# masnottuh/point-cloud-toolbox

Measured on AMD Instinct MI355X. Metric: points/sec curvature (1M-pt torus, k=50); HBM GB/s k-NN vs peak, higher is better.
Workload: dtype f64

## Files before the change

### point-cloud-toolbox_amd/csrc/pct_knn.hip

```cpp
#include "pct_knn_sweep.h"

namespace {

constexpr unsigned kPadElem = 0xFFFFFFFFu;

template <int R>
struct FastK {
    unsigned e[R];
};

__device__ __forceinline__ unsigned umed3(unsigned a, unsigned b, unsigned c) {
    unsigned r;
    asm("v_med3_u32 %0, %1, %2, %3" : "=v"(r) : "v"(a), "v"(b), "v"(c));
    return r;
}

struct SortLanes {
    unsigned sel[6];
    int a31, a63;
};

__device__ __forceinline__ SortLanes make_sort_lanes() {
    SortLanes c;
    const int lane = lane_id();
// ... 1887 lines not shown
        if (a.stats && lane == 0) atomicAdd(&a.counters[4], (unsigned long long)cnt);
    }
}

__global__ __launch_bounds__(256) void k_plain_records(const float* __restrict__ xyz, int64_t n, float4* __restrict__ out) {
    const int64_t i = (int64_t)blockIdx.x * 256 + threadIdx.x;
    if (i < n) out[i] = make_float4(xyz[3 * i], xyz[3 * i + 1], xyz[3 * i + 2], __int_as_float((int)i));
}

template <int R>
__global__ __launch_bounds__(64 * kWavesPerBlock) void k_query_points(const float4* __restrict__ pts, int n, const double* __restrict__ q_xyz,
                                                                      int64_t m, int k, double eps2, int* __restrict__ idx_out,
                                                                      double* __restrict__ dist_out) {
    __shared__ double s_pend_d[kWavesPerBlock][64 * R + 64];
    __shared__ int s_pend_p[kWavesPerBlock][64 * R + 64];
    const int w = __builtin_amdgcn_readfirstlane(threadIdx.x >> 6);
    const int lane = lane_id();
    const int64_t q = (int64_t)blockIdx.x * kWavesPerBlock + w;
    if (q >= m) return;
    Sweep<R> sw;
    sw.k = k - 1;
    sw.eps2 = eps2;
    sw.pts = pts;
    sw.pend_d = s_pend_d[w];
    sw.pend_p = s_pend_p[w];
    sw.qx = q_xyz[3 * q]; sw.qy = q_xyz[3 * q + 1]; sw.qz = q_xyz[3 * q + 2];
    sw.reset();
    for (int base = 0;; base += 64) {
        const bool have = base < n;
        if (have) {
            const int pos = base + lane;
            const bool valid = pos < n;
            float4 c = make_float4(0.f, 0.f, 0.f, 0.f);
            if (valid) c = pts[pos];
            sw.consider(c, pos, valid);
            if (sw.npend < 64 * R) continue;
        }
        if (sw.npend > 0 || sw.empty) sw.flush();
        if (!have) break;
    }
#pragma unroll
    for (int r = 0; r < R; ++r) {
        const int i = lane + 64 * r;
        if (i < k) {
            const bool real = sw.best.p[r] != INT_MAX;
            idx_out[q * k + i] = real ? sw.best.p[r] : n;
            dist_out[q * k + i] = real ? sqrt(sw.best.d[r]) : (double)INFINITY;
        }
    }
}

__device__ __forceinline__ float table_distance(const float4* pts, const double4* ptsd, int qpos, const float4 c) {
    double qx, qy, qz;
    if (ptsd) { const double4 q = ptsd[qpos]; qx = q.x; qy = q.y; qz = q.z; }
    else { const float4 q = pts[qpos]; qx = (double)q.x; qy = (double)q.y; qz = (double)q.z; }
    const double dx = (double)c.x - qx, dy = (double)c.y - qy, dz = (double)c.z - qz;
    return (float)sqrt((dx * dx + dy * dy) + dz * dz);
}

__global__ __launch_bounds__(256) void k_export(const float4* __restrict__ pts, const double4* __restrict__ ptsd, const int* __restrict__ owned_pos, int q_begin,
                                                const int* __restrict__ nbr_pos, const float* __restrict__ nbr_dist,
                                                const int* __restrict__ nbr_cnt, int64_t n, int64_t n_rows, int k, int pitch,
                                                int64_t begin, int64_t end, int* __restrict__ idx_out,
                                                float* __restrict__ dist_out, int* __restrict__ cnt_out) {
    const int64_t t = (int64_t)blockIdx.x * 256 + threadIdx.x;
    const int64_t row = t / k;
    const int j = (int)(t - row * k);
    if (row >= n_rows) return;
    const int pub = owned_pos ? __float_as_int(pts[owned_pos[row]].w) : (int)row + q_begin;
    if (pub < begin || pub >= end) return;
    const int64_t o = (int64_t)(pub - begin) * k + j;
    const int pos = nbr_pos[row * pitch + j];
    const float4 c = pos < 0 ? make_float4(0.f, 0.f, 0.f, 0.f) : pts[pos];
    if (idx_out) idx_out[o] = pos < 0 ? (int)n : __float_as_int(c.w);
    if (dist_out) dist_out[o] = nbr_dist ? nbr_dist[row * pitch + j] : pos < 0 ? INFINITY : table_distance(pts, ptsd, owned_pos[row], c);
    if (cnt_out && j == 0) cnt_out[pub - begin] = nbr_cnt ? nbr_cnt[row] : k;
}

__global__ __launch_bounds__(128) void k_export_rows(const float4* __restrict__ pts, const double4* __restrict__ ptsd, const int* __restrict__ row_of, const int* __restrict__ owned_pos, int q_begin,
                                                     const int* __restrict__ nbr_pos, const float* __restrict__ nbr_dist,
                                                     const int* __restrict__ nbr_cnt, int64_t n, int k, int pitch,
                                                     const int64_t* __restrict__ rows, int* __restrict__ idx_out,
                                                     float* __restrict__ dist_out, int* __restrict__ cnt_out) {
    const int64_t r = blockIdx.x;
    const int64_t pub = rows[r];
    const int64_t row = row_of ? row_of[pub - q_begin] : pub - q_begin;
    for (int j = threadIdx.x; j < k; j += 128) {
        const int pos = nbr_pos[row * pitch + j];
        const float4 c = pos < 0 ? make_float4(0.f, 0.f, 0.f, 0.f) : pts[pos];
        if (idx_out) idx_out[r * k + j] = pos < 0 ? (int)n : __float_as_int(c.w);
        if (dist_out) dist_out[r * k + j] = nbr_dist ? nbr_dist[row * pitch + j] : pos < 0 ? INFINITY : table_distance(pts, ptsd, owned_pos[row], c);
    }
    if (cnt_out && threadIdx.x == 0) cnt_out[r] = nbr_cnt ? nbr_cnt[row] : k;
}

__global__ __launch_bounds__(64) void k_selftest(int* fails) {
    const int lane = lane_id();
    const int v = lane * 7919 + 13;
    int bad = 0;
    bad += lane_xor<1>(v) != __shfl_xor(v, 1);
    bad += lane_xor<2>(v) != __shfl_xor(v, 2);
    bad += lane_xor<4>(v) != __shfl_xor(v, 4);
    bad += lane_xor<8>(v) != __shfl_xor(v, 8);
    bad += lane_xor<16>(v) != __shfl_xor(v, 16);
    bad += lane_xor<32>(v) != __shfl_xor(v, 32);
    if (bad) atomicAdd(fails, bad);
}

__global__ __launch_bounds__(256) void k_item_census(const int2* __restrict__ items, int64_t n_items, int items_q,
                                                     const int* __restrict__ cs, const int* __restrict__ cell_own, pct_grid g, int k,
                                                     int cap, unsigned long long* __restrict__ out) {
    __shared__ unsigned long long sh[4][4];
    unsigned long long v[4] = {0, 0, 0, 0};
    for (int64_t it = (int64_t)blockIdx.x * 256 + threadIdx.x; it < n_items; it += (int64_t)gridDim.x * 256) {
        const int2 e = items[it];
        const int cell = e.x;
        const int cx = cell % g.nx, cy = (cell / g.nx) % g.ny, cz = cell / (g.nx * g.ny);
        const int nq = min(items_q, cell_own[cell] - e.y * items_q);
        int m = 0, occupied = 0;
        for (int dz = -1; dz <= 1; ++dz)
            for (int dy = -1; dy <= 1; ++dy) {
                const int z = cz + dz, y = cy + dy;
                if (z < 0 || z >= g.nz || y < 0 || y >= g.ny) continue;
                const int row = (z * g.ny + y) * g.nx;
                int prev = cs[row + max(cx - 1, 0)];
                for (int x = max(cx - 1, 0); x <= min(cx + 1, g.nx - 1); ++x) {
                    const int next = cs[row + x + 1];
                    occupied += next > prev;
                    m += next - prev;
                    prev = next;
                }
            }
        v[0] += (unsigned)nq;
        if (m > cap) v[1] += (unsigned)nq;
        else if (2 * m < 5 * (k + 1)) v[2] += (unsigned)nq;
        else v[3] += (unsigned long long)nq * (unsigned)occupied;
    }
    for (int j = 0; j < 4; ++j) {
        for (int o = 32; o > 0; o >>= 1) v[j] += __shfl_xor(v[j], o);
        if ((threadIdx.x & 63) == 0) sh[threadIdx.x >> 6][j] = v[j];
    }
    __syncthreads();
    if (threadIdx.x < 4) atomicAdd(&out[threadIdx.x], sh[0][threadIdx.x] + sh[1][threadIdx.x] + sh[2][threadIdx.x] + sh[3][threadIdx.x]);
}

KnnArgs make_args(pct_ctx* ctx, int32_t k, double eps, bool grid) {
    KnnArgs a = {};
    a.pts = (const float4*)(grid ? ctx->sorted4.p : ctx->pts4.p);
    a.ptsd = ctx->has_f64 ? (const double4*)(grid ? ctx->sorted4d.p : ctx->pts4d.p) : nullptr;
    a.cell_start = (const int*)ctx->cell_cnt.p;
    a.cell_own = (const int*)ctx->cell_own.p;
    a.own_start = (const int*)ctx->own_start.p;
    a.owned_pos = (const int*)ctx->owned_pos.p;
    a.n_owned = ctx->own_flag ? ctx->own_count : ctx->q_end - ctx->q_begin;
    a.occ = (const int*)ctx->occ.p;
    a.n_occ = ctx->n_occ;
    a.n = ctx->n;
    a.g = ctx->grid;
    a.k = k;
    a.pitch = (k + 3) & ~3;
    a.eps2 = eps > 0 ? eps * eps : INFINITY;
    a.q_begin = (int)ctx->q_begin;
    a.q_end = (int)ctx->q_end;
    a.nbr_pos = (int*)ctx->nbr_pos.p;
    a.nbr_dist = (float*)ctx->nbr_dist.p;
    a.nbr_cnt = eps > 0 ? (int*)ctx->nbr_cnt.p : nullptr;
    a.row_done = ctx->own_flag || ctx->level_mode ? (int*)ctx->row_done.p : nullptr;
    a.redo_m = a.row_done ? (int*)ctx->redo_m.p : nullptr;
    a.counters = (unsigned long long*)ctx->counters.p;
    a.stats = ctx->collect_stats ? 1 : 0;
    return a;
}

int reserve_table(pct_ctx* ctx, int32_t k, double eps, bool with_dist = true) {
    ctx->nbr_pitch = (k + 3) & ~3;
    const size_t rows = (size_t)(ctx->own_flag ? ctx->own_count : ctx->q_end - ctx->q_begin);
    PCT_TRY(pct_reserve(ctx, &ctx->nbr_pos, rows * ctx->nbr_pitch * sizeof(int)));
    if (with_dist) PCT_TRY(pct_reserve(ctx, &ctx->nbr_dist, rows * ctx->nbr_pitch * sizeof(float)));
    ctx->dist_valid = with_dist;
    if (eps > 0) PCT_TRY(pct_reserve(ctx, &ctx->nbr_cnt, rows * sizeof(int)));
    PCT_TRY(pct_reserve(ctx, &ctx->counters, 64 * sizeof(unsigned long long)));
    if (!ctx->counters_clean) PCT_HIP(ctx, hipMemsetAsync(ctx->counters.p, 0, 64, ctx->stream));
    ctx->counters_clean = false;
    return PCT_OK;
}

}

int pct_launch_knn_grid(pct_ctx* ctx, int32_t k, double eps, bool exact_only, int phase) {
    const int64_t n_rows = ctx->own_flag ? ctx->own_count : ctx->q_end - ctx->q_begin;
    const double c2_ = ctx->grid.cell * ctx->grid.cell;
    const bool f32_ok_ = c2_ > 1e-30 && c2_ < 1e30 && (!(eps > 0) || eps * eps > 1e-36);
    const pct_grid& gg_ = ctx->grid;
    const double far_ = fmax(fmax(fabs(gg_.ox), fabs(gg_.ox + gg_.nx * gg_.cell)),
                             fmax(fmax(fabs(gg_.oy), fabs(gg_.oy + gg_.ny * gg_.cell)), fmax(fabs(gg_.oz), fabs(gg_.oz + gg_.nz * gg_.cell))));
    const bool q64_ok_ = !ctx->has_f64 || far_ * 0x1p-23 < gg_.cell * 0x1p-7;
    const bool pair_kernel = !exact_only && phase == 0 && q64_ok_ && f32_ok_ && !ctx->own_flag && !ctx->level_mode && ctx->n_items > 0 &&
                             k + 1 <= pct_fast_r1_max() && ctx->n_items < ((int64_t)1 << 31) - 8 && !pct_getenv("PCT_NO_PAIR") &&
                             !pct_getenv("PCT_NO_PAIR_KERNEL");
    const bool duo_kernel = !exact_only && phase == 0 && q64_ok_ && f32_ok_ && !ctx->own_flag && !ctx->level_mode && ctx->n_items > 0 &&
                            k + 1 > pct_fast_r1_max() && k + 1 <= 128 && ctx->n_items < ((int64_t)1 << 31) - 8 &&
                            !pct_getenv("PCT_NO_PAIR") && !pct_getenv("PCT_NO_DUO_KERNEL");
    const bool skip_dist = (pair_kernel || duo_kernel) && ctx->skip_dist_req && !pct_getenv("PCT_KEEP_DIST");
    if (phase != 2) {
        PCT_TRY(reserve_table(ctx, k, eps, !skip_dist));
        PCT_TRY(pct_reserve(ctx, &ctx->redo, ((size_t)n_rows + 16) * sizeof(int)));
        if (ctx->level_mode) PCT_TRY(pct_reserve(ctx, &ctx->redo_m, ((size_t)n_rows + 16) * sizeof(int)));
    }
    KnnArgs a = make_args(ctx, k, eps, true);
    if (!ctx->dist_valid) a.nbr_dist = nullptr;
    int* redo_count = (int*)ctx->counters.p + 14;
    int* redo = (int*)ctx->redo.p;
    const dim3 block(64 * kWavesPerBlock);
    if (!exact_only && phase != 2 && ctx->n_items > 0) {
        const dim3 grid1((unsigned)((ctx->n_items + kFastWaves<1> - 1) / kFastWaves<1>)), block1(64 * kFastWaves<1>);
        const dim3 grid2((unsigned)((ctx->n_items + kFastWaves<2> - 1) / kFastWaves<2>)), block2(64 * kFastWaves<2>);
        const int2* items = (const int2*)ctx->occ.p;
        const double c2 = ctx->grid.cell * ctx->grid.cell;
        const bool f32_ok = c2 > 1e-30 && c2 < 1e30 && (!(eps > 0) || eps * eps > 1e-36);
        const pct_grid& gg = ctx->grid;
        const double far = fmax(fmax(fabs(gg.ox), fabs(gg.ox + gg.nx * gg.cell)),
                                fmax(fmax(fabs(gg.oy), fabs(gg.oy + gg.ny * gg.cell)), fmax(fabs(gg.oz), fabs(gg.oz + gg.nz * gg.cell))));
        const bool q64_ok = ctx->has_f64 && f32_ok && far * 0x1p-23 < gg.cell * 0x1p-7 && !ctx->level_mode;
        const bool e = eps > 0, pre = !ctx->has_f64 && f32_ok, r1 = k + 1 <= pct_fast_r1_max();
#define PCT_FAST(R_, E_, P_, GRID_, BLOCK_) \
    PCT_LAUNCH((k_knn_fast<R_, E_, P_>), GRID_, BLOCK_, 0, ctx->stream, a, items, ctx->n_items, ctx->items_q, redo, redo_count)
        const bool no_pair = pct_getenv("PCT_NO_PAIR") != nullptr;
#define PCT_FAST_PAIR(R_, E_, GRID_, BLOCK_) \
    PCT_LAUNCH((k_knn_fast<R_, E_, true, true>), GRID_, BLOCK_, 0, ctx->stream, a, items, ctx->n_items, ctx->items_q, redo, redo_count)
#define PCT_FAST_PAIR64(R_, E_, GRID_, BLOCK_) \
    PCT_LAUNCH((k_knn_fast<R_, E_, true, true, true>), GRID_, BLOCK_, 0, ctx->stream, a, items, ctx->n_items, ctx->items_q, redo, redo_count)
        if (pair_kernel || duo_kernel) {
            PairArgs pa = {};
            pa.pts = a.pts; pa.ptsd = a.ptsd; pa.cell_start = a.cell_start; pa.cell_own = a.cell_own; pa.own_start = a.own_start;
            pa.items = items;
            pa.nbr_pos = a.nbr_pos; pa.nbr_dist = a.nbr_dist; pa.nbr_cnt = a.nbr_cnt;
            pa.redo = redo; pa.redo_count = redo_count; pa.counters = a.counters;
            pa.n_items = (int)ctx->n_items; pa.items_q = ctx->items_q;
            pa.k = a.k; pa.pitch = a.pitch; pa.stats = a.stats; pa.eps2 = a.eps2; pa.g = a.g;
            const auto magic = [](unsigned d, unsigned* mg, int* sh) {
                int l = 0;
                while ((1ull << l) < d) ++l;
                *sh = 30 + l;
                *mg = (unsigned)(((1ull << *sh) + d - 1) / d);
            };
            magic((unsigned)a.g.nx, &pa.magic_x, &pa.shift_x);
            magic((unsigned)a.g.nx * (unsigned)a.g.ny, &pa.magic_xy, &pa.shift_xy);
            pa.items_per_xcd = (int)((ctx->n_items + 7) / 8);
            if (pct_getenv("PCT_NO_XCD_MAP")) pa.items_per_xcd = 0;
            const int64_t n_blk = pa.items_per_xcd ? (int64_t)pa.items_per_xcd * 8 : ctx->n_items;
            const dim3 gridp((unsigned)((n_blk + kPairWaves - 1) / kPairWaves)), blockp(64 * kPairWaves);
            if (duo_kernel) {
                const dim3 gridd((unsigned)n_blk), blockd(64);
                if (ctx->has_f64) {
                    if (e && skip_dist) PCT_LAUNCH((k_knn_duo<true, false, true>), gridd, blockd, 0, ctx->stream, pa);
                    else if (e) PCT_LAUNCH((k_knn_duo<true, true, true>), gridd, blockd, 0, ctx->stream, pa);
                    else if (skip_dist) PCT_LAUNCH((k_knn_duo<false, false, true>), gridd, blockd, 0, ctx->stream, pa);
                    else PCT_LAUNCH((k_knn_duo<false, true, true>), gridd, blockd, 0, ctx->stream, pa);
                } else
                if (e && skip_dist) PCT_LAUNCH((k_knn_duo<true, false>), gridd, blockd, 0, ctx->stream, pa);
                else if (e) PCT_LAUNCH((k_knn_duo<true, true>), gridd, blockd, 0, ctx->stream, pa);
                else if (skip_dist) PCT_LAUNCH((k_knn_duo<false, false>), gridd, blockd, 0, ctx->stream, pa);
                else PCT_LAUNCH((k_knn_duo<false, true>), gridd, blockd, 0, ctx->stream, pa);
            } else
            if (ctx->has_f64) {
                if (e && skip_dist) PCT_LAUNCH((k_knn_pair<true, false, true>), gridp, blockp, 0, ctx->stream, pa);
                else if (e) PCT_LAUNCH((k_knn_pair<true, true, true>), gridp, blockp, 0, ctx->stream, pa);
                else if (skip_dist) PCT_LAUNCH((k_knn_pair<false, false, true>), gridp, blockp, 0, ctx->stream, pa);
                else PCT_LAUNCH((k_knn_pair<false, true, true>), gridp, blockp, 0, ctx->stream, pa);
            } else
            if (e && skip_dist) PCT_LAUNCH((k_knn_pair<true, false>), gridp, blockp, 0, ctx->stream, pa);
            else if (e) PCT_LAUNCH((k_knn_pair<true, true>), gridp, blockp, 0, ctx->stream, pa);
            else if (skip_dist) PCT_LAUNCH((k_knn_pair<false, false>), gridp, blockp, 0, ctx->stream, pa);
            else PCT_LAUNCH((k_knn_pair<false, true>), gridp, blockp, 0, ctx->stream, pa);
        } else
        if (q64_ok && !no_pair) {
            if (r1 && !e) PCT_FAST_PAIR64(1, false, grid1, block1);
            else if (r1) PCT_FAST_PAIR64(1, true, grid1, block1);
            else if (!e) PCT_FAST_PAIR64(2, false, grid2, block2);
            else PCT_FAST_PAIR64(2, true, grid2, block2);
        } else
        if (r1 && !e && pre && !no_pair) PCT_FAST_PAIR(1, false, grid1, block1);
        else if (r1 && e && pre && !no_pair) PCT_FAST_PAIR(1, true, grid1, block1);
        else if (!r1 && !e && pre && !no_pair) PCT_FAST_PAIR(2, false, grid2, block2);
        else if (!r1 && e && pre && !no_pair) PCT_FAST_PAIR(2, true, grid2, block2);
        else if (r1 && !e && pre) PCT_FAST(1, false, true, grid1, block1);
        else if (r1 && e && pre) PCT_FAST(1, true, true, grid1, block1);
        else if (r1 && !e) PCT_FAST(1, false, false, grid1, block1);
        else if (r1) PCT_FAST(1, true, false, grid1, block1);
        else if (!e && pre) PCT_FAST(2, false, true, grid2, block2);
        else if (e && pre) PCT_FAST(2, true, true, grid2, block2);
        else if (!e) PCT_FAST(2, false, false, grid2, block2);
        else PCT_FAST(2, true, false, grid2, block2);
#undef PCT_FAST
#undef PCT_FAST_PAIR
#undef PCT_FAST_PAIR64
        PCT_HIP(ctx, hipGetLastError());
    }
    PCT_HIP(ctx, hipEventRecord(ctx->ev[7], ctx->stream));
    if (phase != 1) {
        const int64_t waves = exact_only ? n_rows : 32768;
        const int blocks = (int)((waves + kWavesPerBlock - 1) / kWavesPerBlock);
        const int* list = exact_only ? nullptr : redo;
        if (k + 1 <= 64)
            PCT_LAUNCH(k_knn_exact<1>, dim3(blocks), block, 0, ctx->stream, a, list, (const int*)redo_count);
        else if (k + 1 <= 128)
            PCT_LAUNCH(k_knn_exact<2>, dim3(blocks), block, 0, ctx->stream, a, list, (const int*)redo_count);
        else
            PCT_TRY(pct_launch_knn_exact_wide(ctx, a, blocks, list, (const int*)redo_count));
        PCT_HIP(ctx, hipGetLastError());
    }
    ctx->knn_sorted_space = true;
    return PCT_OK;
}

int pct_launch_knn_tree(pct_ctx* ctx, int32_t k, double eps) {
    if (ctx->level_mode || ctx->own_flag || ctx->q_begin != 0 || ctx->q_end != ctx->n)
        return pct_fail(ctx, PCT_ERR_INVALID, "the tree sweep takes whole clouds");
    const int64_t n_rows = ctx->n;
    const bool lean_ok = ctx->n_items > 0 && ctx->n_items < ((int64_t)1 << 31) - 8 && !pct_getenv("PCT_NO_PAIR") &&
                         !pct_getenv("PCT_TREE_EXACT_ONLY");
    const bool pair_tree = lean_ok && k + 1 <= pct_fast_r1_max() && !pct_getenv("PCT_NO_PAIR_KERNEL");
    const bool duo_tree = lean_ok && k + 1 > pct_fast_r1_max() && k + 1 <= 128 && !pct_getenv("PCT_NO_DUO_KERNEL");
    const bool skip_dist = (pair_tree || duo_tree) && ctx->skip_dist_req && !pct_getenv("PCT_KEEP_DIST");
    PCT_TRY(reserve_table(ctx, k, eps, !skip_dist));
    PCT_TRY(pct_reserve(ctx, &ctx->redo, ((size_t)n_rows + 16) * sizeof(int)));
    KnnArgs a = make_args(ctx, k, eps, true);
    if (!ctx->dist_valid) a.nbr_dist = nullptr;
    a.tree_seg = (const int4*)ctx->tree_seg.p;
    a.tree_runs = (const int2*)ctx->tree_runs.p;
    a.tree_bits = ctx->tree_bits;
    a.tree_codes = (const unsigned long long*)ctx->tree_codes.p + ctx->n;
    a.tree_lvl = (const unsigned char*)ctx->tree_lvl.p;
    a.tree_bucket = (const int*)ctx->tree_bucket.p;
    int* redo_count = (int*)ctx->counters.p + 14;
    int* redo = (int*)ctx->redo.p;
    const int2* items = (const int2*)ctx->occ.p;
    const bool r1 = k + 1 <= pct_fast_r1_max();
    const bool exact_only = pct_getenv("PCT_TREE_EXACT_ONLY") != nullptr;
    if (ctx->n_items > 0 && !exact_only) {
        const dim3 grid1((unsigned)((ctx->n_items + kFastWaves<1> - 1) / kFastWaves<1>)), block1(64 * kFastWaves<1>);
        const dim3 grid2((unsigned)((ctx->n_items + kFastWaves<2> - 1) / kFastWaves<2>)), block2(64 * kFastWaves<2>);
        const bool e = eps > 0;
#define PCT_TREE(R_, E_, Q_, GRID_, BLOCK_) \
    PCT_LAUNCH((k_knn_fast<R_, E_, true, true, Q_, true>), GRID_, BLOCK_, 0, ctx->stream, a, items, ctx->n_items, ctx->items_q, redo, redo_count)
        if (pair_tree || duo_tree) {
            PairArgs pa = {};
            pa.pts = a.pts; pa.ptsd = a.ptsd; pa.cell_start = a.cell_start;
            pa.items = items;
            pa.nbr_pos = a.nbr_pos; pa.nbr_dist = a.nbr_dist; pa.nbr_cnt = a.nbr_cnt;
            pa.redo = redo; pa.redo_count = redo_count; pa.counters = a.counters;
            pa.n_items = (int)ctx->n_items; pa.items_q = ctx->items_q;
            pa.k = a.k; pa.pitch = a.pitch; pa.stats = a.stats; pa.eps2 = a.eps2; pa.g = a.g;
            pa.tree_seg = a.tree_seg; pa.tree_runs = a.tree_runs; pa.tree_bits = a.tree_bits;
            pa.items_per_xcd = pct_getenv("PCT_NO_XCD_MAP") ? 0 : (int)((ctx->n_items + 7) / 8);
            const int64_t n_blk = pa.items_per_xcd ? (int64_t)pa.items_per_xcd * 8 : ctx->n_items;
            const dim3 gridp((unsigned)((n_blk + kPairWaves - 1) / kPairWaves)), blockp(64 * kPairWaves);
#define PCT_PAIR_TREE(E_, D_, Q_)                                                                       \
    do {                                                                                                \
        if (duo_tree) PCT_LAUNCH((k_knn_duo<E_, D_, Q_, true>), dim3((unsigned)n_blk), dim3(64), 0, ctx->stream, pa); \
        else PCT_LAUNCH((k_knn_pair<E_, D_, Q_, true>), gridp, blockp, 0, ctx->stream, pa);           \
    } while (0)
            if (ctx->has_f64) {
                if (e && skip_dist) PCT_PAIR_TREE(true, false, true);
                else if (e) PCT_PAIR_TREE(true, true, true);
                else if (skip_dist) PCT_PAIR_TREE(false, false, true);
                else PCT_PAIR_TREE(false, true, true);
            } else if (e && skip_dist) PCT_PAIR_TREE(true, false, false);
            else if (e) PCT_PAIR_TREE(true, true, false);
            else if (skip_dist) PCT_PAIR_TREE(false, false, false);
            else PCT_PAIR_TREE(false, true, false);
#undef PCT_PAIR_TREE
        } else
        if (ctx->has_f64) {
            if (r1 && !e) PCT_TREE(1, false, true, grid1, block1);
            else if (r1) PCT_TREE(1, true, true, grid1, block1);
            else if (!e) PCT_TREE(2, false, true, grid2, block2);
            else PCT_TREE(2, true, true, grid2, block2);
        } else if (r1 && !e) PCT_TREE(1, false, false, grid1, block1);
        else if (r1) PCT_TREE(1, true, false, grid1, block1);
        else if (!e) PCT_TREE(2, false, false, grid2, block2);
        else PCT_TREE(2, true, false, grid2, block2);
#undef PCT_TREE
        PCT_HIP(ctx, hipGetLastError());
    }
    PCT_HIP(ctx, hipEventRecord(ctx->ev[7], ctx->stream));
    const int blocks = (32768 + kWavesPerBlock - 1) / kWavesPerBlock;
    const int* list = exact_only ? nullptr : redo;
    if (k + 1 <= 64)
        PCT_LAUNCH(k_knn_exact_tree<1>, dim3(blocks), dim3(64 * kWavesPerBlock), 0, ctx->stream, a, list, (const int*)redo_count);
    else
        PCT_LAUNCH(k_knn_exact_tree<2>, dim3(blocks), dim3(64 * kWavesPerBlock), 0, ctx->stream, a, list, (const int*)redo_count);
    PCT_HIP(ctx, hipGetLastError());
    ctx->knn_sorted_space = true;
    return PCT_OK;
}

int pct_item_census(pct_ctx* ctx, int32_t k, unsigned long long out4[4]) {
    PCT_TRY(pct_reserve(ctx, &ctx->counters, 64 * sizeof(unsigned long long)));
    PCT_HIP(ctx, hipMemsetAsync(ctx->counters.p, 0, 64, ctx->stream));
    ctx->counters_clean = false;
    const int cap = k + 1 <= pct_fast_r1_max() ? kStageCap : PCT_STAGE_CAP2_HOST;
    const int blocks = (int)((ctx->n_items + 255) / 256 < 1024 ? (ctx->n_items + 255) / 256 : 1024);
    if (blocks > 0) {
        PCT_LAUNCH(k_item_census, dim3(blocks), dim3(256), 0, ctx->stream, (const int2*)ctx->occ.p, ctx->n_items, ctx->items_q,
                           (const int*)ctx->cell_cnt.p, (const int*)ctx->cell_own.p, ctx->grid, k, cap, (unsigned long long*)ctx->counters.p);
        PCT_HIP(ctx, hipGetLastError());
    }
    PCT_HIP(ctx, hipMemcpyAsync(ctx->pin + 2112, ctx->counters.p, 32, hipMemcpyDeviceToHost, ctx->stream));
    PCT_HIP(ctx, hipStreamSynchronize(ctx->stream));
    memcpy(out4, ctx->pin + 2112, 32);
    return PCT_OK;
}

int pct_launch_knn_brute(pct_ctx* ctx, int32_t k, double eps) {
    PCT_TRY(reserve_table(ctx, k, eps));
    KnnArgs a = make_args(ctx, k, eps, false);
    const int64_t nq = ctx->q_end - ctx->q_begin;
    const int blocks = (int)((nq + kWavesPerBlock - 1) / kWavesPerBlock);
    if (blocks > 0) {
        if (k + 1 <= 64)
            PCT_LAUNCH(k_knn_brute<1>, dim3(blocks), dim3(64 * kWavesPerBlock), 0, ctx->stream, a);
        else if (k + 1 <= 128)
            PCT_LAUNCH(k_knn_brute<2>, dim3(blocks), dim3(64 * kWavesPerBlock), 0, ctx->stream, a);
        else
            PCT_TRY(pct_launch_knn_brute_wide(ctx, a, blocks));
        PCT_HIP(ctx, hipGetLastError());
    }
    ctx->knn_sorted_space = false;
    return PCT_OK;
}

int pct_launch_export_neighbors(pct_ctx* ctx, int64_t begin, int64_t end, int32_t* d_idx, float* d_dist,
                                int32_t* d_cnt) {
    const bool sorted = ctx->knn_sorted_space;
    const int64_t n_rows = ctx->q_end - ctx->q_begin;
    const int64_t total = n_rows * ctx->k;
    const int blocks = (int)((total + 255) / 256);
    PCT_LAUNCH(k_export, dim3(blocks), dim3(256), 0, ctx->stream,
                       (const float4*)(sorted ? ctx->sorted4.p : ctx->pts4.p), sorted && ctx->has_f64 ? (const double4*)ctx->sorted4d.p : nullptr,
                       sorted ? (const int*)ctx->owned_pos.p : nullptr,
                       (int)ctx->q_begin, (const int*)ctx->nbr_pos.p, ctx->dist_valid ? (const float*)ctx->nbr_dist.p : nullptr,
                       ctx->eps > 0 ? (const int*)ctx->nbr_cnt.p : nullptr, ctx->n, n_rows, ctx->k, ctx->nbr_pitch, begin, end,
                       d_idx, d_dist, d_cnt);
    PCT_HIP(ctx, hipGetLastError());
    return PCT_OK;
}

int pct_launch_export_rows(pct_ctx* ctx, const int64_t* d_rows, int64_t n_rows, int32_t* d_idx, float* d_dist, int32_t* d_cnt) {
    const bool sorted = ctx->knn_sorted_space;
    if (sorted) PCT_TRY(pct_ensure_row_of(ctx));
    PCT_LAUNCH(k_export_rows, dim3((unsigned)n_rows), dim3(128), 0, ctx->stream,
                       (const float4*)(sorted ? ctx->sorted4.p : ctx->pts4.p), sorted && ctx->has_f64 ? (const double4*)ctx->sorted4d.p : nullptr,
                       sorted ? (const int*)ctx->row_of.p : nullptr,
                       sorted ? (const int*)ctx->owned_pos.p : nullptr,
                       (int)ctx->q_begin, (const int*)ctx->nbr_pos.p, ctx->dist_valid ? (const float*)ctx->nbr_dist.p : nullptr,
                       ctx->eps > 0 ? (const int*)ctx->nbr_cnt.p : nullptr, ctx->n, ctx->k, ctx->nbr_pitch, d_rows, d_idx,
                       d_dist, d_cnt);
    PCT_HIP(ctx, hipGetLastError());
    return PCT_OK;
}

int pct_ensure_plain_records(pct_ctx* ctx) {
    if (!ctx->qpts4_valid) {
        PCT_TRY(pct_reserve(ctx, &ctx->qpts4, (size_t)ctx->n * sizeof(float4)));
        PCT_LAUNCH(k_plain_records, dim3((unsigned)((ctx->n + 255) / 256)), dim3(256), 0, ctx->stream,
                           ctx->xyz_view, ctx->n, (float4*)ctx->qpts4.p);
        PCT_HIP(ctx, hipGetLastError());
        ctx->qpts4_valid = true;
    }
    return PCT_OK;
}

int pct_launch_query_points(pct_ctx* ctx, const double* d_q, int64_t m, int32_t k, double eps, int32_t* d_idx, double* d_dist) {
    PCT_TRY(pct_ensure_plain_records(ctx));
    const double eps2 = eps > 0 ? eps * eps : (double)INFINITY;
    const int blocks = (int)((m + kWavesPerBlock - 1) / kWavesPerBlock);
    if (k <= 64)
        PCT_LAUNCH(k_query_points<1>, dim3(blocks), dim3(64 * kWavesPerBlock), 0, ctx->stream,
                           (const float4*)ctx->qpts4.p, (int)ctx->n, d_q, m, k, eps2, d_idx, d_dist);
    else
        PCT_LAUNCH(k_query_points<2>, dim3(blocks), dim3(64 * kWavesPerBlock), 0, ctx->stream,
                           (const float4*)ctx->qpts4.p, (int)ctx->n, d_q, m, k, eps2, d_idx, d_dist);
    PCT_HIP(ctx, hipGetLastError());
    return PCT_OK;
}

int pct_launch_selftest(pct_ctx* ctx, int* d_fails) {
    PCT_LAUNCH(k_selftest, dim3(1), dim3(64), 0, ctx->stream, d_fails);
    PCT_HIP(ctx, hipGetLastError());
    return PCT_OK;
}
```

### point-cloud-toolbox_amd/csrc/pct_knn_sweep.h

```cpp
#pragma once
#include "pct_internal.h"

#include <math.h>
#include <type_traits>

struct KnnArgs {
    const float4* pts;
    const double4* ptsd;
    const int* cell_start;
    const int* cell_own;
    const int* own_start;
    const int* owned_pos;
    int64_t n_owned;
    const int* occ;
    int64_t n_occ;
    int64_t n;
    pct_grid g;
    int k;
    int pitch;
    double eps2;
    int q_begin, q_end;
    int* nbr_pos;
    float* nbr_dist;
    int* nbr_cnt;
    int* row_done;
    int* redo_m;
    const int4* tree_seg;
    const int2* tree_runs;
    int tree_bits;
    const unsigned long long* tree_codes;
    const unsigned char* tree_lvl;
    const int* tree_bucket;
    int stats;
    unsigned long long* counters;
};

int pct_launch_knn_exact_wide(pct_ctx* ctx, const KnnArgs& a, int blocks, const int* list, const int* list_count);
int pct_launch_knn_brute_wide(pct_ctx* ctx, const KnnArgs& a, int blocks);

namespace {

constexpr int kWavesPerBlock = 4;
#ifndef PCT_STAGE_CAP
#define PCT_STAGE_CAP 512
#endif
constexpr int kStageCap = PCT_STAGE_CAP;
#ifndef PCT_STAGE_CAP2
#define PCT_STAGE_CAP2 768
#endif
constexpr int PCT_STAGE_CAP2_HOST = PCT_STAGE_CAP2;
#ifndef PCT_TREE_CAP
#define PCT_TREE_CAP 768
#endif
#ifndef PCT_TREE_CAP2
#define PCT_TREE_CAP2 1024
#endif


__device__ __forceinline__ int lane_id() { return threadIdx.x & 63; }

__device__ __forceinline__ void wave_lds_sync() {
    __builtin_amdgcn_fence(__ATOMIC_RELEASE, "wavefront");
    __builtin_amdgcn_wave_barrier();
    __builtin_amdgcn_fence(__ATOMIC_ACQUIRE, "wavefront");
}

template <int S>
__device__ __forceinline__ int lane_xor(int v) {
    if constexpr (S == 1) {
        return __builtin_amdgcn_mov_dpp(v, 0xB1, 0xF, 0xF, true);
    } else if constexpr (S == 2) {
        return __builtin_amdgcn_mov_dpp(v, 0x4E, 0xF, 0xF, true);
    } else if constexpr (S == 4) {
        int t = __builtin_amdgcn_update_dpp(v, v, 0x124, 0xF, 0xA, false);
        return __builtin_amdgcn_update_dpp(t, v, 0x12C, 0xF, 0x5, false);
    } else if constexpr (S == 8) {
        return __builtin_amdgcn_mov_dpp(v, 0x128, 0xF, 0xF, true);
    } else if constexpr (S == 16) {
        const auto r = __builtin_amdgcn_permlane16_swap((unsigned)v, (unsigned)v, false, false);
        return (int)((threadIdx.x & 16) ? r[0] : r[1]);
    } else {
        const auto r = __builtin_amdgcn_permlane32_swap((unsigned)v, (unsigned)v, false, false);
        return (int)((threadIdx.x & 32) ? r[0] : r[1]);
    }
}

__device__ __forceinline__ int pub_index(const float4* pts, int pos) { return __float_as_int(pts[pos].w); }

__device__ __forceinline__ bool key_less(double da, int pa, double db, int pb, const float4* pts) {
    const bool lt = da < db;
    bool tie = (da == db) && (pa != pb) && (pa != INT_MAX) && (pb != INT_MAX);
    bool tb = false;
    if (__builtin_expect(__ballot(tie) != 0ull, 0)) {
        if (tie) tb = pub_index(pts, pa) < pub_index(pts, pb);
    }
    return lt || (tie && tb);
}

template <int R>
struct TopK {
    double d[R];
    int p[R];
};

template <int R, int STRIDE>
__device__ __forceinline__ void bitonic_level(TopK<R>& t, int size, bool descending, const float4* pts) {
    const int lane = lane_id();
    if constexpr (STRIDE >= 64) {
        constexpr int ds = STRIDE >> 6;
#pragma unroll
        for (int r = 0; r < R; ++r) {
            if ((r & ds) == 0 && (r | ds) < R) {
                const int r2 = r | ds;
                const int i = lane + 64 * r;
                const bool asc = ((i & size) == 0) != descending;
                const bool hi_less = key_less(t.d[r2], t.p[r2], t.d[r], t.p[r], pts);
                if (hi_less == asc) {
                    double td = t.d[r]; t.d[r] = t.d[r2]; t.d[r2] = td;
                    int tp = t.p[r]; t.p[r] = t.p[r2]; t.p[r2] = tp;
                }
            }
        }
    } else {
#pragma unroll
        for (int r = 0; r < R; ++r) {
            const int lo = lane_xor<STRIDE>(__double2loint(t.d[r]));
            const int hi = lane_xor<STRIDE>(__double2hiint(t.d[r]));
            const int pp = lane_xor<STRIDE>(t.p[r]);
            const double pd = __hiloint2double(hi, lo);
            const int i = lane + 64 * r;
            const bool asc = ((i & size) == 0) != descending;
            const bool keep_min = ((lane & STRIDE) == 0) == asc;
            const bool partner_less = key_less(pd, pp, t.d[r], t.p[r], pts);
            if (keep_min == partner_less) {
                t.d[r] = pd;
                t.p[r] = pp;
            }
        }
    }
}

template <int R, int STRIDE>
__device__ __forceinline__ void bitonic_strides(TopK<R>& t, int size, bool descending, const float4* pts) {
    bitonic_level<R, STRIDE>(t, size, descending, pts);
    if constexpr (STRIDE > 1) bitonic_strides<R, STRIDE / 2>(t, size, descending, pts);
}

template <int R, int SIZE>
__device__ __forceinline__ void bitonic_sort_from(TopK<R>& t, bool descending, const float4* pts) {
    bitonic_strides<R, SIZE / 2>(t, SIZE, descending, pts);
    if constexpr (SIZE < 64 * R) bitonic_sort_from<R, SIZE * 2>(t, descending, pts);
}

template <int R>
__device__ __forceinline__ void bitonic_merge_min(TopK<R>& best, const TopK<R>& batch, const float4* pts) {
#pragma unroll
    for (int r = 0; r < R; ++r) {
        if (key_less(batch.d[r], batch.p[r], best.d[r], best.p[r], pts)) {
            best.d[r] = batch.d[r];
            best.p[r] = batch.p[r];
        }
    }
    bitonic_strides<R, 32 * R>(best, 64 * R, false, pts);
}

template <int R>
struct Sweep {
    TopK<R> best;
    double tau_d;
    int tau_p;
    int npend;
    bool empty;
    double qx, qy, qz;
    double eps2;
    int k;
    const float4* pts;
    double* pend_d;
    int* pend_p;

    __device__ __forceinline__ void reset() {
#pragma unroll
        for (int r = 0; r < R; ++r) {
            best.d[r] = INFINITY;
            best.p[r] = INT_MAX;
        }
        tau_d = INFINITY;
        tau_p = INT_MAX;
        npend = 0;
        empty = true;
    }

    __device__ __forceinline__ void refresh_tau() {
        const int slot = k >> 6, src = k & 63;
        double d = best.d[0];
        int p = best.p[0];
#pragma unroll
        for (int r = 1; r < R; ++r)
            if (slot == r) { d = best.d[r]; p = best.p[r]; }
        tau_d = __shfl(d, src);
        tau_p = __shfl(p, src);
    }

    __device__ __forceinline__ void flush() {
        const int lane = lane_id();
        TopK<R> b;
        wave_lds_sync();
        const int take = npend < 64 * R ? npend : 64 * R;
#pragma unroll
        for (int r = 0; r < R; ++r) {
            const int i = lane + 64 * r;
            const bool v = i < take;
            b.d[r] = v ? pend_d[i] : INFINITY;
            b.p[r] = v ? pend_p[i] : INT_MAX;
        }
        const int rest = npend - take;
        double md = 0;
        int mp = 0;
        if (lane < rest) { md = pend_d[take + lane]; mp = pend_p[take + lane]; }
        wave_lds_sync();
        if (lane < rest) { pend_d[lane] = md; pend_p[lane] = mp; }
        wave_lds_sync();
        npend = rest;
        bitonic_sort_from<R, 2>(b, !empty, pts);
        if (empty) {
            best = b;
            empty = false;
        } else {
            bitonic_merge_min<R>(best, b, pts);
        }
        refresh_tau();
    }

    __device__ __forceinline__ void consider(float4 c, int pos, bool valid) {
        const double dx = (double)c.x - qx, dy = (double)c.y - qy, dz = (double)c.z - qz;
        const double d2 = (dx * dx + dy * dy) + dz * dz;
        const bool closer = key_less(d2, valid ? pos : INT_MAX, tau_d, tau_p, pts);
        const bool pass = valid && d2 < eps2 && closer;
        const unsigned long long m = __ballot(pass);
        if (pass) {
            const int slot = npend + __builtin_amdgcn_mbcnt_hi((unsigned)(m >> 32), __builtin_amdgcn_mbcnt_lo((unsigned)m, 0));
            pend_d[slot] = d2;
            pend_p[slot] = pos;
        }
        npend += __popcll(m);
    }

    __device__ __forceinline__ void store(int64_t row, int pitch, int* nbr_pos, float* nbr_dist, int* nbr_cnt) {
        const int lane = lane_id();
        int found = 0;
#pragma unroll
        for (int r = 0; r < R; ++r) {
            const int i = lane + 64 * r;
            const bool real = best.p[r] != INT_MAX;
            if (i >= 1 && i <= k) {
                nbr_pos[row * pitch + (i - 1)] = real ? best.p[r] : -1;
                if (nbr_dist) nbr_dist[row * pitch + (i - 1)] = real ? (float)sqrt(best.d[r]) : INFINITY;
                found += real;
            }
        }
        if (nbr_cnt) {
            for (int o = 32; o > 0; o >>= 1) found += __shfl_xor(found, o);
            if (lane == 0) nbr_cnt[row] = found;
        }
    }
};

__constant__ signed char kRowOrder[9][2] = {{0, 0}, {0, -1}, {0, 1}, {-1, 0}, {1, 0}, {-1, -1}, {-1, 1}, {1, -1}, {1, 1}};

struct ShellIter {
    int r_lo, ring, zlo, ylo, wy, nrows, row, part, pos, end, chunk;
    unsigned long long live;
    int b_s0, b_e0, b_s1, b_e1;
    double prune, gx, gy, gz, slack;
    __device__ __forceinline__ void start(const pct_grid& g, int cy, int cz, int lo, int hi, double prune_d2 = INFINITY,
                                          double qgx = 0.0, double qgy = 0.0, double qgz = 0.0) {
        const double ce = g.cell * (1.0 - 1e-6);
        prune = prune_d2 / (ce * ce);
        gx = qgx; gy = qgy; gz = qgz;
        slack = 1e-15 * ((double)g.nx + (double)g.ny + (double)g.nz + fabs(qgx) + fabs(qgy) + fabs(qgz));
        r_lo = lo; ring = hi;
        zlo = max(-hi, -cz);
        ylo = max(-hi, -cy);
        const int zhi = min(hi, g.nz - 1 - cz), yhi = min(hi, g.ny - 1 - cy);
        wy = yhi - ylo + 1;
        nrows = (zhi - zlo + 1) * wy;
        row = 0; part = 0; pos = 0; end = 0; chunk = -1; live = 0ull;
    }
    __device__ __forceinline__ void fetch(const pct_grid& g, const int* __restrict__ cs, int cx, int cy, int cz) {
        const int ri = chunk + lane_id();
        b_s0 = b_e0 = b_s1 = b_e1 = 0;
        if (ri < nrows) {
            const int dz = zlo + ri / wy, dy = ylo + ri % wy;
            const int base = ((cz + dz) * g.ny + (cy + dy)) * g.nx;
            const bool inner = max(abs(dz), abs(dy)) <= r_lo;
            int x_lo = -ring, x_hi = ring;
            if (prune < INFINITY) {
                const double ty = dy > 0 ? fmax(dy - gy - slack, 0.0) : dy < 0 ? fmax(gy - (dy + 1) - slack, 0.0) : 0.0;
                const double tz = dz > 0 ? fmax(dz - gz - slack, 0.0) : dz < 0 ? fmax(gz - (dz + 1) - slack, 0.0) : 0.0;
                const double left = prune - (ty * ty + tz * tz);
                if (left < 0.0) { x_lo = 1; x_hi = 0; }
                else {
                    const double rx = sqrt(left) * (1.0 + 1e-9) + 1e-9 + slack;
                    x_hi = (int)fmin((double)ring, floor(rx + gx));
                    x_lo = -(int)fmin((double)ring, floor(rx + 1.0 - gx));
                    x_hi = max(x_hi, 0);
                    x_lo = min(x_lo, 0);
                }
            }
            if (x_lo <= x_hi) {
                if (!inner) {
                    b_s0 = cs[base + max(cx + x_lo, 0)];
                    b_e0 = cs[base + min(cx + x_hi, g.nx - 1) + 1];
                } else {
                    const int a0 = max(cx + x_lo, 0), a1 = cx - r_lo - 1;
                    const int c0 = cx + r_lo + 1, c1 = min(cx + x_hi, g.nx - 1);
                    if (a1 >= a0) { b_s0 = cs[base + a0]; b_e0 = cs[base + a1 + 1]; }
                    if (c1 >= c0) { b_s1 = cs[base + c0]; b_e1 = cs[base + c1 + 1]; }
                }
            }
        }
        live = __builtin_amdgcn_ballot_w64(b_e0 > b_s0 || b_e1 > b_s1);
    }
    __device__ __forceinline__ bool next(const pct_grid& g, const int* __restrict__ cs, int cx, int cy, int cz, int& base, int& lim) {
        while (pos >= end) {
            if (row >= nrows) return false;
            if (chunk < 0 || row - chunk >= 64) { chunk = row; fetch(g, cs, cx, cy, cz); }
            int l = row - chunk;
            if (part == 0) {
                const unsigned long long rest = live >> l;
                if (rest == 0ull) { row = chunk + 64; continue; }
                const int skip = (int)__builtin_ctzll(rest);
                row += skip;
                l += skip;
                pos = __builtin_amdgcn_readlane(b_s0, l);
                end = __builtin_amdgcn_readlane(b_e0, l);
                part = 1;
            } else {
                pos = __builtin_amdgcn_readlane(b_s1, l);
                end = __builtin_amdgcn_readlane(b_e1, l);
                part = 0;
                ++row;
            }
        }
        base = pos;
        lim = end;
        pos += 64;
        return true;
    }
};

__device__ __forceinline__ double guaranteed_r2(const pct_grid& g, int cx, int cy, int cz, double gx, double gy, double gz, int ring) {
    const double inf = INFINITY;
    double gmin = inf;
    gmin = fmin(gmin, cx - ring <= 0 ? inf : gx + ring);
    gmin = fmin(gmin, cx + ring >= g.nx - 1 ? inf : (1.0 - gx) + ring);
    gmin = fmin(gmin, cy - ring <= 0 ? inf : gy + ring);
    gmin = fmin(gmin, cy + ring >= g.ny - 1 ? inf : (1.0 - gy) + ring);
    gmin = fmin(gmin, cz - ring <= 0 ? inf : gz + ring);
    gmin = fmin(gmin, cz + ring >= g.nz - 1 ? inf : (1.0 - gz) + ring);
    const double rr = gmin * g.cell * (1.0 - 1e-6);
    return rr * rr;
}

__device__ __forceinline__ double limit_r2(const pct_grid& g, int cx, int cy, int cz, double gx, double gy, double gz) {
    const double px = cx + gx, py = cy + gy, pz = cz + gz;
    double t = fmin(px - g.lim_lo[0], g.lim_hi[0] - px);
    t = fmin(t, fmin(py - g.lim_lo[1], g.lim_hi[1] - py));
    t = fmin(t, fmin(pz - g.lim_lo[2], g.lim_hi[2] - pz));
    const double rr = fmax(t, 0.0) * g.cell * (1.0 - 1e-6);
    return rr * rr;
}

__device__ __forceinline__ int cell_coord_d(double x, double o, double inv, int n) {
    int c = (int)floor((x - o) * inv);
    return min(max(c, 0), n - 1);
}

template <int R>
__global__ __launch_bounds__(64 * kWavesPerBlock) void k_knn_exact(KnnArgs a, const int* __restrict__ list,
                                                                   const int* __restrict__ list_count) {
    __shared__ double s_pend_d[kWavesPerBlock][64 * R + 64];
    __shared__ int s_pend_p[kWavesPerBlock][64 * R + 64];
    const int w = __builtin_amdgcn_readfirstlane(threadIdx.x >> 6);
    const int lane = lane_id();
    const pct_grid g = a.g;
    const int* __restrict__ cs = a.cell_start;
    const int64_t total = list ? (int64_t)*list_count : a.n_owned;
    const int64_t nwaves = (int64_t)gridDim.x * kWavesPerBlock;

    Sweep<R> sw;
    sw.k = a.k;
    sw.eps2 = a.eps2;
    sw.pts = a.pts;
    sw.pend_d = s_pend_d[w];
    sw.pend_p = s_pend_p[w];

    for (int64_t item = (int64_t)blockIdx.x * kWavesPerBlock + w; item < total; item += nwaves) {
        const int row = list ? list[item] : (int)item;
        const int q = a.owned_pos[row];
        const float4 qp = a.pts[q];
        const int cx = __builtin_amdgcn_readfirstlane(cell_coord_d((double)qp.x, g.ox, g.inv_cell, g.nx));
        const int cy = __builtin_amdgcn_readfirstlane(cell_coord_d((double)qp.y, g.oy, g.inv_cell, g.ny));
        const int cz = __builtin_amdgcn_readfirstlane(cell_coord_d((double)qp.z, g.oz, g.inv_cell, g.nz));
        if (a.ptsd) {
            const double4 qd = a.ptsd[q];
            sw.qx = qd.x; sw.qy = qd.y; sw.qz = qd.z;
        } else {
            sw.qx = (double)qp.x; sw.qy = (double)qp.y; sw.qz = (double)qp.z;
        }
        sw.reset();
        const double gx = (sw.qx - g.ox) * g.inv_cell - cx;
        const double gy = (sw.qy - g.oy) * g.inv_cell - cy;
        const double gz = (sw.qz - g.oz) * g.inv_cell - cz;
        ShellIter it;
        it.start(g, cy, cz, -1, 1);
        int nbase = 0, nlim = 0;
        bool have_next = it.next(g, cs, cx, cy, cz, nbase, nlim);
        float4 c_next = make_float4(0.f, 0.f, 0.f, 0.f);
        if (have_next && nbase + lane < nlim) c_next = a.pts[nbase + lane];
        for (;;) {
            const bool have = have_next;
            if (have) {
                const int pos = nbase + lane;
                const bool valid = pos < nlim;
                const float4 c = c_next;
                have_next = it.next(g, cs, cx, cy, cz, nbase, nlim);
                if (have_next && nbase + lane < nlim) c_next = a.pts[nbase + lane];
                sw.consider(c, pos, valid);
                if (sw.npend < 64 * R) continue;
            }
            if (sw.npend > 0 || sw.empty) sw.flush();
            if (have) continue;
            if (fmin(sw.tau_d, sw.eps2) <= guaranteed_r2(g, cx, cy, cz, gx, gy, gz, it.ring)) {
                if (lane == 0 && fmin(sw.tau_d, sw.eps2) > limit_r2(g, cx, cy, cz, gx, gy, gz)) atomicAdd(&a.counters[5], 1ull);
                break;
            }
            it.start(g, cy, cz, it.ring, it.ring < 4 ? it.ring + 1 : it.ring + (it.ring + 1) / 2, fmin(sw.tau_d, sw.eps2), gx, gy, gz);
            have_next = it.next(g, cs, cx, cy, cz, nbase, nlim);
            if (have_next && nbase + lane < nlim) c_next = a.pts[nbase + lane];
        }
        if (a.stats && lane == 0 && it.ring > 1) atomicAdd(&a.counters[0], 1ull);
        sw.store(row, a.pitch, a.nbr_pos, a.nbr_dist, a.nbr_cnt);
        if (a.row_done && lane == 0) a.row_done[row] = 1;
    }
}

template <int R>
__global__ __launch_bounds__(64 * kWavesPerBlock) void k_knn_exact_tree(KnnArgs a, const int* __restrict__ list,
                                                                        const int* __restrict__ list_count) {
    __shared__ double s_pend_d[kWavesPerBlock][64 * R + 64];
    __shared__ int s_pend_p[kWavesPerBlock][64 * R + 64];
    const int w = __builtin_amdgcn_readfirstlane(threadIdx.x >> 6);
    const int lane = lane_id();
    const int64_t total = list ? (int64_t)*list_count : a.n_owned;
    const int64_t nwaves = (int64_t)gridDim.x * kWavesPerBlock;

    Sweep<R> sw;
    sw.k = a.k;
    sw.eps2 = a.eps2;
    sw.pts = a.pts;
    sw.pend_d = s_pend_d[w];
    sw.pend_p = s_pend_p[w];

    for (int64_t item = (int64_t)blockIdx.x * kWavesPerBlock + w; item < total; item += nwaves) {
        const int row = list ? list[item] : (int)item;
        if (a.ptsd) {
            const double4 qd = a.ptsd[row];
            sw.qx = qd.x; sw.qy = qd.y; sw.qz = qd.z;
        } else {
            const float4 qp = a.pts[row];
            sw.qx = (double)qp.x; sw.qy = (double)qp.y; sw.qz = (double)qp.z;
        }
        const unsigned long long code = a.tree_codes[row];
        const int fx = (int)pct_compact3(code), fy = (int)pct_compact3(code >> 1), fz = (int)pct_compact3(code >> 2);
        int level = __builtin_amdgcn_readfirstlane((int)a.tree_lvl[row]);
        int rounds = 0;
        unsigned long long steps = 0;
        for (;;) {
            pct_grid g = a.g;
            g.cell = __builtin_ldexp(a.g.cell, level);
            g.inv_cell = __builtin_ldexp(a.g.inv_cell, -level);
            g.nx = g.ny = g.nz = 1 << (a.tree_bits - level);
            const int cx = __builtin_amdgcn_readfirstlane(fx >> level), cy = __builtin_amdgcn_readfirstlane(fy >> level),
                      cz = __builtin_amdgcn_readfirstlane(fz >> level);
            int run_s = 0, run_len = 0;
            if (lane < 27) {
                int dx, dy, dz;
                pct_stencil_cell(lane, &dx, &dy, &dz);
                const int x = cx + dx, y = cy + dy, z = cz + dz;
                if (x >= 0 && x < g.nx && y >= 0 && y < g.ny && z >= 0 && z < g.nz) {
                    const unsigned long long prefix = pct_spread3((unsigned)x) | pct_spread3((unsigned)y) << 1 | pct_spread3((unsigned)z) << 2;
                    const int64_t lo = pct_code_lower_bound(a.tree_codes, a.tree_bucket, prefix << (3 * level));
                    const int64_t hi = pct_code_lower_bound(a.tree_codes, a.tree_bucket, (prefix + 1) << (3 * level));
                    run_s = (int)lo;
                    run_len = (int)(hi - lo);
                }
            }
            sw.reset();
            for (int t = 0; t < 27; ++t) {
                const int s0 = __builtin_amdgcn_readlane(run_s, t), s1 = s0 + __builtin_amdgcn_readlane(run_len, t);
                for (int base = s0; base < s1; base += 64) {
                    const int pos = base + lane;
                    const bool valid = pos < s1;
                    float4 c = make_float4(0.f, 0.f, 0.f, 0.f);
                    if (valid) c = a.pts[pos];
                    sw.consider(c, pos, valid);
                    if (sw.npend >= 64 * R) sw.flush();
                    ++steps;
                }
            }
            if (sw.npend > 0 || sw.empty) sw.flush();
            const double gx = (sw.qx - g.ox) * g.inv_cell - cx;
            const double gy = (sw.qy - g.oy) * g.inv_cell - cy;
            const double gz = (sw.qz - g.oz) * g.inv_cell - cz;
            if (fmin(sw.tau_d, sw.eps2) <= guaranteed_r2(g, cx, cy, cz, gx, gy, gz, 1) || level >= a.tree_bits) break;
            ++level;
            ++rounds;
        }
        if (a.stats && lane == 0) {
            if (rounds > 0) atomicAdd(&a.counters[0], 1ull);
            atomicAdd(&a.counters[3], steps);
            atomicMax(&a.counters[6], (steps << 32) | (unsigned)row);
        }
        sw.store(row, a.pitch, a.nbr_pos, a.nbr_dist, a.nbr_cnt);
    }
}

template <int R>
__global__ __launch_bounds__(64 * kWavesPerBlock) void k_knn_brute(KnnArgs a) {
    __shared__ double s_pend_d[kWavesPerBlock][64 * R + 64];
    __shared__ int s_pend_p[kWavesPerBlock][64 * R + 64];
    const int w = __builtin_amdgcn_readfirstlane(threadIdx.x >> 6);
    const int lane = lane_id();
    const int64_t q = (int64_t)a.q_begin + (int64_t)blockIdx.x * kWavesPerBlock + w;
    if (q >= a.q_end) return;

    Sweep<R> sw;
    sw.k = a.k;
    sw.eps2 = a.eps2;
    sw.pts = a.pts;
    sw.pend_d = s_pend_d[w];
    sw.pend_p = s_pend_p[w];
    if (a.ptsd) {
        const double4 qd = a.ptsd[q];
        sw.qx = qd.x; sw.qy = qd.y; sw.qz = qd.z;
    } else {
        const float4 qp = a.pts[q];
        sw.qx = (double)qp.x; sw.qy = (double)qp.y; sw.qz = (double)qp.z;
    }
    sw.reset();
    const int n = (int)a.n;
    for (int base = 0;; base += 64) {
        const bool have = base < n;
        if (have) {
            const int pos = base + lane;
            const bool valid = pos < n;
            float4 c = make_float4(0.f, 0.f, 0.f, 0.f);
            if (valid) c = a.pts[pos];
            sw.consider(c, pos, valid);
            if (sw.npend < 64 * R) continue;
        }
        if (sw.npend > 0 || sw.empty) sw.flush();
        if (!have) break;
    }
    sw.store(q - a.q_begin, a.pitch, a.nbr_pos, a.nbr_dist, a.nbr_cnt);
}

}
```

Baseline: 1.414 billion.

## Split redo-row first-cube scan across a block's waves with shared-memory top-k merge

For the exact k-NN redo pass, each redo row is now handled by a whole block instead of a single wave. The four waves split the first shell's cell chunks round-robin, and each keeps a partial top-k. The partial lists are then merged into wave 0 with bitonic merges through shared memory, and wave 0 continues any further rings alone. The goal is to cut tail latency when only a few redo rows remain, at the cost of extra shared memory, a block-wide sync, and idle waves after the first cube. Note that w>0 waves return inside the item loop, so the team path only works if each block handles at most one item, which the total<=gridDim check enforces.

Result: slower. 1.395 billion (-1.4%).

```diff
diff --git a/point-cloud-toolbox_amd/csrc/pct_knn.hip b/point-cloud-toolbox_amd/csrc/pct_knn.hip
--- a/point-cloud-toolbox_amd/csrc/pct_knn.hip
+++ b/point-cloud-toolbox_amd/csrc/pct_knn.hip
@@ -2213,10 +2213,13 @@
         const int64_t waves = exact_only ? n_rows : 32768;
         const int blocks = (int)((waves + kWavesPerBlock - 1) / kWavesPerBlock);
         const int* list = exact_only ? nullptr : redo;
+        KnnArgs ax = a;
+        ax.team = !exact_only && !pct_getenv("PCT_REDO_WAVES");
+        const int team_blocks = ax.team ? 4096 : blocks;
         if (k + 1 <= 64)
-            PCT_LAUNCH(k_knn_exact<1>, dim3(blocks), block, 0, ctx->stream, a, list, (const int*)redo_count);
+            PCT_LAUNCH(k_knn_exact<1>, dim3(team_blocks), block, 0, ctx->stream, ax, list, (const int*)redo_count);
         else if (k + 1 <= 128)
-            PCT_LAUNCH(k_knn_exact<2>, dim3(blocks), block, 0, ctx->stream, a, list, (const int*)redo_count);
+            PCT_LAUNCH(k_knn_exact<2>, dim3(team_blocks), block, 0, ctx->stream, ax, list, (const int*)redo_count);
         else
             PCT_TRY(pct_launch_knn_exact_wide(ctx, a, blocks, list, (const int*)redo_count));
         PCT_HIP(ctx, hipGetLastError());
diff --git a/point-cloud-toolbox_amd/csrc/pct_knn_sweep.h b/point-cloud-toolbox_amd/csrc/pct_knn_sweep.h
--- a/point-cloud-toolbox_amd/csrc/pct_knn_sweep.h
+++ b/point-cloud-toolbox_amd/csrc/pct_knn_sweep.h
@@ -32,6 +32,7 @@
     const unsigned char* tree_lvl;
     const int* tree_bucket;
     int stats;
+    int team;
     unsigned long long* counters;
 };
 
@@ -376,17 +377,86 @@
     return min(max(c, 0), n - 1);
 }
 
+constexpr int kTeamSteps = 6;
+constexpr int kTeamMaxR = 2;
+
+template <int R, int J>
+__device__ __forceinline__ void team_consider(Sweep<R>& sw, const float4 (&c)[kTeamSteps], const int (&pos)[kTeamSteps],
+                                              unsigned valid, unsigned used) {
+    if constexpr (J < kTeamSteps) {
+        if (used >> J & 1u) {
+            sw.consider(c[J], pos[J], (valid >> J & 1u) != 0u);
+            if (sw.npend >= 64 * R) sw.flush();
+        }
+        team_consider<R, J + 1>(sw, c, pos, valid, used);
+    }
+}
+
+template <int R>
+__device__ __forceinline__ void team_first_cube(Sweep<R>& sw, ShellIter& it, const KnnArgs& a, const pct_grid& g,
+                                                const int* __restrict__ cs, int cx, int cy, int cz, int w,
+                                                double* __restrict__ m_d, int* __restrict__ m_p) {
+    const int lane = lane_id();
+    int step = 0;
+    bool more = true;
+    while (more) {
+        float4 c[kTeamSteps];
+        int pos[kTeamSteps];
+        unsigned valid = 0u, used = 0u;
+#pragma unroll
+        for (int j = 0; j < kTeamSteps; ++j) {
+            int base = 0, lim = 0;
+            c[j] = make_float4(0.f, 0.f, 0.f, 0.f);
+            while (more) {
+                int b = 0, l = 0;
+                more = it.next(g, cs, cx, cy, cz, b, l);
+                if (!more) break;
+                if ((step++ & (kWavesPerBlock - 1)) == w) { base = b; lim = l; break; }
+            }
+            pos[j] = base + lane;
+            if (lim > base) used |= 1u << j;
+            if (pos[j] < lim) { valid |= 1u << j; c[j] = a.pts[pos[j]]; }
+        }
+        team_consider<R, 0>(sw, c, pos, valid, used);
+    }
+    if (sw.npend > 0 || sw.empty) sw.flush();
+    if (w > 0) {
+#pragma unroll
+        for (int r = 0; r < R; ++r) {
+            m_d[(w - 1) * 64 * R + lane + 64 * r] = sw.best.d[r];
+            m_p[(w - 1) * 64 * R + lane + 64 * r] = sw.best.p[r];
+        }
+    }
+    __syncthreads();
+    if (w > 0) return;
+    for (int o = 0; o < kWavesPerBlock - 1; ++o) {
+        TopK<R> b;
+#pragma unroll
+        for (int r = 0; r < R; ++r) {
+            const int i = 64 * R - 1 - (lane + 64 * r);
+            b.d[r] = m_d[o * 64 * R + i];
+            b.p[r] = m_p[o * 64 * R + i];
+        }
+        bitonic_merge_min<R>(sw.best, b, sw.pts);
+    }
+    sw.refresh_tau();
+}
+
 template <int R>
 __global__ __launch_bounds__(64 * kWavesPerBlock) void k_knn_exact(KnnArgs a, const int* __restrict__ list,
                                                                    const int* __restrict__ list_count) {
     __shared__ double s_pend_d[kWavesPerBlock][64 * R + 64];
     __shared__ int s_pend_p[kWavesPerBlock][64 * R + 64];
+    constexpr bool kTeam = R <= kTeamMaxR;
+    __shared__ double s_merge_d[kTeam ? (kWavesPerBlock - 1) * 64 * R : 1];
+    __shared__ int s_merge_p[kTeam ? (kWavesPerBlock - 1) * 64 * R : 1];
     const int w = __builtin_amdgcn_readfirstlane(threadIdx.x >> 6);
     const int lane = lane_id();
     const pct_grid g = a.g;
     const int* __restrict__ cs = a.cell_start;
     const int64_t total = list ? (int64_t)*list_count : a.n_owned;
-    const int64_t nwaves = (int64_t)gridDim.x * kWavesPerBlock;
+    const bool team = kTeam && a.team && list && total <= (int64_t)gridDim.x;
+    const int64_t nwaves = team ? (int64_t)gridDim.x : (int64_t)gridDim.x * kWavesPerBlock;
 
     Sweep<R> sw;
     sw.k = a.k;
@@ -395,7 +465,7 @@
     sw.pend_d = s_pend_d[w];
     sw.pend_p = s_pend_p[w];
 
-    for (int64_t item = (int64_t)blockIdx.x * kWavesPerBlock + w; item < total; item += nwaves) {
+    for (int64_t item = team ? (int64_t)blockIdx.x : (int64_t)blockIdx.x * kWavesPerBlock + w; item < total; item += nwaves) {
         const int row = list ? list[item] : (int)item;
         const int q = a.owned_pos[row];
         const float4 qp = a.pts[q];
@@ -415,9 +485,18 @@
         ShellIter it;
         it.start(g, cy, cz, -1, 1);
         int nbase = 0, nlim = 0;
-        bool have_next = it.next(g, cs, cx, cy, cz, nbase, nlim);
+        bool have_next = false;
         float4 c_next = make_float4(0.f, 0.f, 0.f, 0.f);
-        if (have_next && nbase + lane < nlim) c_next = a.pts[nbase + lane];
+        if constexpr (kTeam) {
+            if (team) {
+                team_first_cube<R>(sw, it, a, g, cs, cx, cy, cz, w, s_merge_d, s_merge_p);
+                if (w > 0) return;
+            }
+        }
+        if (!team) {
+            have_next = it.next(g, cs, cx, cy, cz, nbase, nlim);
+            if (have_next && nbase + lane < nlim) c_next = a.pts[nbase + lane];
+        }
         for (;;) {
             const bool have = have_next;
             if (have) {
```
